# casys-kaist/CoVA

Measured on AMD Instinct MI355X. Metric: compressed-domain frames/sec (BlobNet+bboxcc) at 1080p b=256, higher is better.
Workload: dtype f16

## Files before the change

### cova_amd/csrc/blobnet.h

```cpp
#pragma once
#include <hip/hip_fp16.h>

#include <vector>

#include "internal.h"

constexpr int BN_T = 4;
constexpr int BN_LEVELS = 4;
constexpr int BN_KTAB_STACKS = 256;

struct BnLevelGeom {
    int H, W;
};

struct BnWorkspace {
    bool ready = false;
    __half *act[BN_LEVELS + 1] = {};
    __half *dact[BN_LEVELS] = {};
    __half *pbuf = nullptr;
    size_t pbuf_frames = 0;
    float *part = nullptr;
    int32_t *d_index = nullptr;
    int32_t *h_index = nullptr;
    size_t index_ints = 0;
    hipEvent_t ev_index = nullptr;
    std::vector<int32_t> last_table;
    int last_n_frames = 0;
};

struct covahip_blobnet {
    int H = 0, W = 0, max_batch = 0;
    BnLevelGeom lv[BN_LEVELS + 1];
    int enc_c[BN_LEVELS + 1] = {3, 16, 32, 64, 128};
    int dec_ci[BN_LEVELS] = {128, 128, 64, 32};
    int dec_co[BN_LEVELS] = {64, 32, 16, 16};
    int dec_cy[BN_LEVELS], dec_cx[BN_LEVELS];
    BnWorkspace ws[COVAHIP_MAX_LANES];
    void *d_prepared = nullptr;
    size_t prepared_bytes = 0;
    struct Prepared *prep = nullptr;
    int fuse_tail = 1;
    int fuse_dec = 1;
    int enc1_tile16 = 1;
    int tail_rows = 1;
    int tail_part = 1;
    int fuse_enc23 = 1;
    int enc_rowtiles = 1;
    int64_t macs_per_frame = 0;
};

constexpr int BN_E1_MAXW = 62;
inline bool bn_level1_on_enc1(const covahip_ctx *ctx, const covahip_blobnet *m) {
    return m->enc1_tile16 && m->enc_c[1] == 16 && m->enc_c[2] == 32 && m->lv[1].W <= BN_E1_MAXW && m->lv[1].H >= 2 &&
           !ctx->enc_plan[1].nbands;
}

int blobnet_prepare_mfma(covahip_ctx *ctx, covahip_blobnet *m, const float *h_weights);
void blobnet_release_mfma(covahip_ctx *ctx, covahip_blobnet *m);
struct BnCcTail {
    int area_thresh, max_boxes;
    covahip_box *boxes;
    int32_t *counts;
};
struct BnInput {
    const uint8_t *stack = nullptr;
    const uint8_t *frames = nullptr;
    int n_frames = 0;
    const int32_t *index = nullptr;
    const int32_t *h_index = nullptr;
    bool packed = false;
    bool dry = false;
};
int blobnet_forward_mfma(covahip_ctx *ctx, covahip_blobnet *m, BnWorkspace &ws, const BnInput &in, int batch, float *d_logits,
                         uint8_t *d_mask, const BnCcTail *cc = nullptr, bool *cc_done = nullptr);
```

### cova_amd/csrc/blobnet.hip

```cpp
#include <algorithm>
#include <cstdlib>
#include <cstring>
#include <vector>

#include "blobnet.h"
#include "covahip_dev.h"

namespace {

constexpr uint32_t W_MAGIC = 0x57485643;
constexpr size_t N_PARAMS = 320305;

}

static void free_model(covahip_ctx *ctx, covahip_blobnet *m) {
    if (!m) return;
    blobnet_release_mfma(ctx, m);
    for (BnWorkspace &ws : m->ws) {
        for (int i = 0; i <= BN_LEVELS; i++)
            if (ws.act[i]) hipFree(ws.act[i]);
        for (int j = 0; j < BN_LEVELS; j++)
            if (ws.dact[j]) hipFree(ws.dact[j]);
        if (ws.pbuf) hipFree(ws.pbuf);
        if (ws.part) hipFree(ws.part);
// ... 180 lines not shown
        plan.n_frames = (pass & 2) ? b + BN_T - 1 : 0;
        rc = blobnet_forward_mfma(ctx, m, m->ws[0], plan, b, nullptr, nullptr, nullptr, nullptr);
    }
    return rc;
}

extern "C" {

int covahip_blobnet_load(covahip_ctx *ctx, const void *weights, size_t weights_bytes, int h_mb, int w_mb, int t,
                         int max_batch) {
    if (!ctx || !weights || h_mb <= 0 || w_mb <= 0 || max_batch <= 0) return COVAHIP_ERR_INVALID_ARG;
    if (t != BN_T) return COVAHIP_ERR_UNSUPPORTED;
    if (h_mb < 16 || w_mb < 16 || h_mb > 1024 || w_mb > 1024) return COVAHIP_ERR_UNSUPPORTED;
    if (weights_bytes < 64) return COVAHIP_ERR_BAD_WEIGHTS;
    uint32_t hdr[16];
    std::memcpy(hdr, weights, 64);
    static const uint32_t want[] = {W_MAGIC, 1, 4, 3, 16, 32, 64, 128, 64, 32, 16, 16, (uint32_t)N_PARAMS};
    for (int i = 0; i < 13; i++)
        if (hdr[i] != want[i]) return COVAHIP_ERR_BAD_WEIGHTS;
    if (weights_bytes != 64 + N_PARAMS * sizeof(float)) return COVAHIP_ERR_BAD_WEIGHTS;
    const float *h_w = reinterpret_cast<const float *>(static_cast<const uint8_t *>(weights) + 64);

    COVAHIP_CHECK_HIP(ctx, hipSetDevice(ctx->device));
    covahip_blobnet_destroy(ctx);
    covahip_blobnet *m = new covahip_blobnet();
    int rc = build_model(ctx, m, h_w, h_mb, w_mb, max_batch);
    if (rc == COVAHIP_OK && hipStreamSynchronize(ctx->stream) != hipSuccess) rc = COVAHIP_ERR_HIP;
    if (rc) {
        hipStreamSynchronize(ctx->stream);
        (void)hipGetLastError();
        free_model(ctx, m);
        return rc;
    }
    ctx->blobnet = m;
    return COVAHIP_OK;
}

int covahip_blobnet_macs_per_frame(covahip_ctx *ctx, int64_t *macs) {
    if (!ctx || !macs) return COVAHIP_ERR_INVALID_ARG;
    if (!ctx->blobnet) return COVAHIP_ERR_NOT_LOADED;
    *macs = ctx->blobnet->macs_per_frame;
    return COVAHIP_OK;
}

int covahip_blobnet_set_enc_plan(covahip_ctx *ctx, int level, int nbands, int nbuf) {
    if (!ctx || level < 1 || level > 3 || nbands < 0 || nbands > 64 || (nbands && nbuf != 1 && nbuf != 2)) return COVAHIP_ERR_INVALID_ARG;
    ctx->enc_plan[level].nbands = nbands;
    ctx->enc_plan[level].nbuf = nbands ? nbuf : 0;
    return COVAHIP_OK;
}

int covahip_blobnet_set_impl(covahip_ctx *ctx, int impl) {
    if (!ctx || !ctx->blobnet) return COVAHIP_ERR_NOT_LOADED;
    if (impl != 1 && (impl < 4 || impl > 10)) return COVAHIP_ERR_INVALID_ARG;
    ctx->blobnet->fuse_dec = impl != 4;
    ctx->blobnet->enc1_tile16 = impl != 5;
    ctx->blobnet->enc_rowtiles = impl != 6;
    ctx->blobnet->fuse_enc23 = impl == 7 ? 0 : impl == 8 ? 2 : 1;
    ctx->blobnet->tail_part = impl != 9;
    ctx->blobnet->tail_rows = impl != 10;
    return COVAHIP_OK;
}

static int filter_placed(covahip_ctx *ctx, covahip_blobnet *m, const uint8_t *d_src, int n_frames, const int32_t *stack_index,
                         int batch, int area_thresh, covahip_box *d_boxes, int32_t *d_counts, int max_boxes, float *d_logits,
                         uint8_t *d_mask, bool packed = false) {
    if (!d_mask) {
        CtxLane &l = ctx->lane();
        int rc = covahip_ensure_buffer(ctx, &l.cc_scratch, &l.cc_scratch_bytes, (size_t)batch * m->H * m->W);
        if (rc) return rc;
        d_mask = (uint8_t *)l.cc_scratch;
    }
    BnInput in;
    if (n_frames > 0) {
        int rc = prepare_frames(ctx, m, m->ws[ctx->cur_lane], d_src, n_frames, stack_index, batch, in);
        if (rc) return rc;
        in.packed = packed;
    } else {
        in.stack = d_src;
    }
    return filter_dev(ctx, in, batch, d_logits, d_mask, true, area_thresh, d_boxes, d_counts, max_boxes);
}

static int filter_any(covahip_ctx *ctx, const uint8_t *src, int n_frames, const int32_t *stack_index, int batch,
                      int area_thresh, covahip_box *boxes, int32_t *counts, int max_boxes, float *logits, uint8_t *mask,
                      int mem_kind) {
    if (!ctx || batch < 0 || max_boxes < 0 || n_frames < 0) return COVAHIP_ERR_INVALID_ARG;
    covahip_blobnet *m = ctx->blobnet;
    if (!m) return COVAHIP_ERR_NOT_LOADED;
    if (batch == 0) return COVAHIP_OK;
    if (!src || !counts || (!boxes && max_boxes > 0) || batch > m->max_batch) return COVAHIP_ERR_INVALID_ARG;
    COVAHIP_CHECK_HIP(ctx, hipSetDevice(ctx->device));
    const bool by_frames = n_frames > 0;
    const size_t hw = (size_t)m->H * m->W;
    const size_t in_bytes = by_frames ? (size_t)n_frames * hw * 4 : (size_t)batch * BN_T * hw * 4;
    const size_t mask_bytes = (size_t)batch * hw;
    const size_t logit_bytes = mask_bytes * sizeof(float);
    const size_t box_bytes = (size_t)batch * max_boxes * sizeof(covahip_box);
    const size_t cnt_bytes = (size_t)batch * sizeof(int32_t);
    auto al = [](size_t x) { return (x + 255) & ~(size_t)255; };
    if (mem_kind != COVAHIP_MEM_DEVICE && mem_kind != COVAHIP_MEM_HOST) return COVAHIP_ERR_INVALID_ARG;

    if (mem_kind == COVAHIP_MEM_DEVICE) {
        LaneScope lane(ctx);
        if (!lane.ok()) return COVAHIP_ERR_HIP;
        return filter_placed(ctx, m, src, n_frames, stack_index, batch, area_thresh, boxes, counts, max_boxes, logits, mask);
    }
    if (int rc = covahip_primary_op(ctx)) return rc;
    const uint8_t *d_src = src;
    int rc = covahip_ensure_buffer(ctx, &ctx->stage_in, &ctx->stage_in_bytes, in_bytes);
    if (rc) return rc;
    rc = covahip_ensure_buffer(ctx, &ctx->stage_out, &ctx->stage_out_bytes,
                               al(mask_bytes) + al(logit_bytes) + al(box_bytes) + al(cnt_bytes));
// ... 170 lines not shown
```

### cova_amd/csrc/blobnet_mfma.hip

```cpp
#include <algorithm>
#include <cmath>
#include <cstdlib>
#include <cstring>
#include <mutex>
#include <type_traits>
#include <utility>
#include <vector>

#include "bboxcc_body.h"
#include "bboxcc_wave.h"
#include "blobnet.h"

typedef _Float16 half8 __attribute__((ext_vector_type(8)));
typedef _Float16 half4 __attribute__((ext_vector_type(4)));
typedef float f32x16 __attribute__((ext_vector_type(16)));
typedef float f32x4 __attribute__((ext_vector_type(4)));
typedef _Float16 half2v __attribute__((ext_vector_type(2)));

namespace {

constexpr float BN_EPS = 1e-3f;
constexpr int WG = 256;

struct EncPrep {
// ... 685 lines not shown
        }
        landed();
        PHASE_MARK(6);
#ifdef WGSPAN_ONLY
        ITEM_MARK(3);
        it_n_++;
#endif
    }
#ifdef WGSPAN_ONLY
    if (tid == 0 && blockIdx.x < 1024)
        for (int i = 0; i < 4; i++)
            for (int j = 0; j < 4; j++) g_itemspan[COUT == 32 ? 0 : COUT == 64 ? 1 : 2][blockIdx.x][i][j] = it_t_[i][j];
#endif
#ifdef PHASE_TIMING
#ifndef PHASE_WAVE
#define PHASE_WAVE 0
#endif
    if (tid == 64 * (PHASE_WAVE < 0 ? NWV + PHASE_WAVE : PHASE_WAVE))
        for (int i = 0; i < 9; i++) atomicAdd(&g_phase[i + (PRE ? 0 : COUT == 64 ? 16 : COUT == 128 ? 32 : 48)], ph_[i]);
#endif
    WGSPAN_END(COUT == 32 ? 0 : COUT == 64 ? 1 : 2);
}

constexpr int E2_TSZ = 16384, E3_TSZ = 26112;
constexpr int E1_RS = 2176;
constexpr int E1_TR = 8;
constexpr int E1_TSZ = E1_RS * E1_TR;
constexpr int E1_MAXW = BN_E1_MAXW;
static_assert(8 * 2 * (E1_MAXW + 2) <= 2 * 512 && (E1_MAXW + 2) * 32 + 32 <= E1_RS, "enc1_mfma's staging / row limits");
struct Enc1Args {
    const __half *in;
    __half *out;
    const half8 *wfrag;
    const float *epi;
    int B, H, W, Hp, Wp, Ho, Wo, oy, ox;
    int nbands;
    uint32_t mWp, mRC;
    int scr_off;
    ItemPlan plan;
    const int32_t *pidx;
    __half *skip;
    const float *tm_pre;
    int use_ktab;
    float *part;
    const half8 *wtail;
    uint32_t mXe;
    uint16_t ktab[BN_KTAB_STACKS * BN_T];
};
constexpr int E1_CONST = 2560;
#ifndef E1_ABL
#define E1_ABL 0
#endif
template <bool ALLPOS>
__global__ __launch_bounds__(512, 4) void enc1_mfma(Enc1Args p) {
    constexpr int NWV = 8, WGS = NWV * 64, MG = NWV;
    constexpr int AD = 4;
    extern __shared__ __attribute__((aligned(16))) uint8_t smem[];
    WGSPAN_BEGIN();
    const int tid = threadIdx.x;
    const int wave = __builtin_amdgcn_readfirstlane(tid >> 6);
    for (int i = tid; i < BN_T * E1_TSZ / 16; i += WGS) *reinterpret_cast<uint4 *>(smem + i * 16) = make_uint4(0, 0, 0, 0);
    uint8_t *const cst = smem + p.scr_off + NWV * 1024;
    if (tid < 96) reinterpret_cast<float *>(cst)[tid] = p.epi[tid];
    if (p.part && tid >= 256 && tid < 384) reinterpret_cast<half8 *>(cst + 512)[tid - 256] = p.wtail[tid - 256];
    if (tid >= 128 && tid < 136) {
        const int i = tid & 3;
        const float *tmw = (tid & 4) ? p.tm_pre : p.epi + 96;
        {
            half4 a1, a2;
#pragma unroll
            for (int t = 0; t < BN_T; t++) { a1[t] = (_Float16)tmw[t * BN_T + i]; a2[t] = (_Float16)tmw[16 + t * BN_T + i]; }
            *reinterpret_cast<half4 *>(cst + 384 + (tid & 4) * 16 + i * 16) = a1;
            *reinterpret_cast<half4 *>(cst + 384 + (tid & 4) * 16 + i * 16 + 8) = a2;
        }
    }
    const int RCr = 2 * (p.W + 2);
    const uint32_t plane = (uint32_t)p.H * p.W * 32;
#ifdef PHASE_TIMING
    unsigned long long ph_[9] = {0, 0, 0, 0, 0, 0, 0, 0, 0}, last_ = __builtin_amdgcn_s_memrealtime();
    asm volatile("s_waitcnt lgkmcnt(0)" ::: "memory");
#endif

    ItemIter it;
    for (bool more = it.start(p.plan, p.B, p.nbands); more; more = it.next(p.plan, p.B, p.nbands)) {
        const int b = it.b, band = it.band;
        const int y0 = 2 * ((band * p.Hp) / p.nbands);
        const int rows = 2 * (((band + 1) * p.Hp) / p.nbands) - y0;
        const int n2 = rows + 2;
        auto lane_id = []() -> int {
            uint32_t zero = 0;
            asm volatile("" : "+v"(zero));
            return (int)__builtin_amdgcn_mbcnt_hi(~0u, __builtin_amdgcn_mbcnt_lo(~0u, zero));
        };
        const int ll = lane_id();
        int fidx[BN_T] = {BN_T * b, BN_T * b + 1, BN_T * b + 2, BN_T * b + 3};
        const uint8_t *const fbase = reinterpret_cast<const uint8_t *>(p.in);
        if (p.use_ktab) {
            typedef unsigned u32x2 __attribute__((ext_vector_type(2)));
            typedef const __attribute__((address_space(4))) u32x2 *const_u32x2_ptr;
            const __attribute__((address_space(4))) uint8_t *ka = (const __attribute__((address_space(4))) uint8_t *)__builtin_amdgcn_kernarg_segment_ptr();
            const u32x2 row = *(const_u32x2_ptr)(ka + offsetof(Enc1Args, ktab) + (size_t)b * 8);
            fidx[0] = row[0] & 0xFFFF; fidx[1] = row[0] >> 16; fidx[2] = row[1] & 0xFFFF; fidx[3] = row[1] >> 16;
        } else if (p.pidx) {
            typedef int i32x4 __attribute__((ext_vector_type(4)));
            typedef const __attribute__((address_space(4))) i32x4 *const_i32x4_ptr;
            const i32x4 row = *(const_i32x4_ptr)(uintptr_t)(p.pidx + b * BN_T);
            fidx[0] = row[0]; fidx[1] = row[1]; fidx[2] = row[2]; fidx[3] = row[3];
// ... 185 lines not shown
                __builtin_amdgcn_sched_group_barrier(0x008, 2, 0);
                if (k + AD < 20) __builtin_amdgcn_sched_group_barrier(0x100, 1, 0);
            }
#if E1_ABL == 3
            asm volatile("" :: "v"(tw.x), "v"(e0[0]), "v"(e1[0]), "v"(e0[1]), "v"(e1[1]));
            continue;
#endif
#ifdef PHASE_TIMING
            asm volatile("" : "+v"(pooled[0]), "+v"(pooled[1]));
            PHASE_MARK(6);
#endif
            TmixW tm;
            tm.a1 = __builtin_bit_cast(half4, make_uint2(tw.x, tw.y));
            tm.a2 = __builtin_bit_cast(half4, make_uint2(tw.z, tw.w));
#pragma unroll
            for (int t = 0; t < BN_T; t++) tm.id[t] = (_Float16)(t == (m & 3) ? 1.f : 0.f);
            half4 pb2[2], o2[2];
#pragma unroll
            for (int nt = 0; nt < 2; nt++) pb2[nt] = __builtin_convertvector(pooled[nt], half4);
            tmix4h<2>(tm, pb2, o2);
#pragma unroll
            for (int nt = 0; nt < 2; nt++) {
                _Float16 *sw = reinterpret_cast<_Float16 *>(scr + kg * 256) + nt * 16 + m;
#pragma unroll
                for (int t = 0; t < BN_T; t++) sw[t * 32] = o2[nt][t];
            }
            __builtin_amdgcn_fence(__ATOMIC_RELEASE, "wavefront");
            __builtin_amdgcn_wave_barrier();
            __builtin_amdgcn_fence(__ATOMIC_ACQUIRE, "wavefront");
            const int owin = tile * 4 + kg;
            const uint4 sv = *reinterpret_cast<const uint4 *>(scr + ll * 16);
            if (owin < nwin) {
                const int owy = fdiv(owin, p.mWp), owx = owin - owy * p.Wp;
                const int gy = y0 / 2 + owy + p.oy, gx = owx + p.ox;
                const uint32_t eo = (uint32_t)((gy * p.Wo + gx) * 32 + 8 * (m & 3));
                *reinterpret_cast<uint4 *>(ob + (m >> 2) * tstride + eo) = sv;
                if (ride && m < 4) {
                    float *const pw = reinterpret_cast<float *>(pb4 + (y0 + 2 * owy) * GW + 2 * owx) + m;
                    pw[0] = pride[0]; pw[4] = pride[1]; pw[4 * GW] = pride[2]; pw[4 * GW + 4] = pride[3];
                }
            }
            __builtin_amdgcn_fence(__ATOMIC_RELEASE, "wavefront");
            __builtin_amdgcn_wave_barrier();
            PHASE_MARK(7);
        }
    }
#ifdef PHASE_TIMING
    if (tid == 64 * (PHASE_WAVE < 0 ? NWV + PHASE_WAVE : PHASE_WAVE))
        for (int i = 0; i < 9; i++) atomicAdd(&g_phase[i], ph_[i]);
#endif
    WGSPAN_END(0);
}

constexpr int E23_RP2 = 2048;
constexpr int E23_NSLOT = 6;
constexpr int E23_TSZ2 = E23_NSLOT * E23_RP2;
struct Enc23Args {
    const __half *in;
    __half *mid;
    __half *out;
    const half8 *wf2, *wf3;
    const float *epi2, *epi3;
    int B;
    int H2, W2, Hp2, Wp2;
    int H3, W3, Hp3, Wp3, oy3, ox3;
    int H4, W4, oy4, ox4;
    Swz swz2, swz3;
    int ring_off, xchg_off, scr_off;
};
template <bool AP2, bool AP3>
__global__ __launch_bounds__(512, 2) void enc23_mfma(Enc23Args p) {
    extern __shared__ __attribute__((aligned(256))) uint8_t smem[];
    WGSPAN_BEGIN();
    const int tid = threadIdx.x, lane = tid & 63;
    const int wave = __builtin_amdgcn_readfirstlane(tid >> 6);
    uint8_t *const ring = smem + p.ring_off;
    uint8_t *const xchg = smem + p.xchg_off;
    const int TC3 = p.W3 + 2;
    bool first = true;
    const int tc2 = wave & 1, nt2 = (wave >> 1) & 1, th = wave >> 2;
    const int nt3 = wave & 3, mg3 = wave >> 2;
    for (int b = blockIdx.x; b < p.B; b += gridDim.x) {
        int ll = lane;
        asm volatile("" : "+v"(ll));
        lds_barrier();
        const uint8_t *const src_b = reinterpret_cast<const uint8_t *>(p.in) + (size_t)b * BN_T * p.H2 * p.W2 * 64;
        const int st_t = tid >> 7, st_i = tid & 127, st_c = st_i >> 2, st_x = st_c - 1;
        const bool st_xin = st_x >= 0 && st_x < p.W2;
        uint32_t st_so[2];
#pragma unroll
        for (int k = 0; k < 2; k++)
            st_so[k] = (uint32_t)((min(max(st_x, 0), p.W2 - 1)) * 64 + (((st_i & 3) ^ swz_eval<4>(p.swz2, st_c, k)) << 4));
        const uint8_t *const st_src = src_b + (size_t)st_t * p.H2 * p.W2 * 64;
        uint8_t *const st_dst = ring + st_t * E23_TSZ2 + st_i * 16;
        auto load_rows = [&](int r0, uint4 (&v)[2]) {
#pragma unroll
            for (int k = 0; k < 2; k++) {
                const int rc = min(max(r0 + k, 0), p.H2 - 1);
                v[k] = *reinterpret_cast<const uint4 *>(st_src + (size_t)rc * p.W2 * 64 + st_so[k]);
            }
        };
        auto store_rows = [&](int r0, const uint4 (&v)[2]) {
#pragma unroll
            for (int k = 0; k < 2; k++) {
                const int row = r0 + k;
                const bool in = st_xin && row >= 0 && row < p.H2;
// ... 1286 lines not shown
                else LAUNCH((enc0p_mfma<false, true>), dim3(grid), dim3(WG0), lds, ctx->stream, a);
            } else {
                if (pr->allpos[0]) LAUNCH((enc0p_mfma<true, false>), dim3(grid), dim3(WG0), lds, ctx->stream, a);
                else LAUNCH((enc0p_mfma<false, false>), dim3(grid), dim3(WG0), lds, ctx->stream, a);
            }
        }
        COVAHIP_CHECK_HIP(ctx, hipGetLastError());
    }
    for (int i = 1; i < BN_LEVELS; i++) {
        const int H = m->lv[i].H, W = m->lv[i].W, Hp = H / 2, Wp = W / 2;
        const int cin = m->enc_c[i];
        if (i == 2 && m->fuse_enc23 && m->enc_rowtiles && !ctx->enc_plan[2].nbands && !ctx->enc_plan[3].nbands && cin == 32 &&
            m->enc_c[3] == 64 && m->enc_c[4] == 128) {
            const int H3 = m->lv[3].H, W3 = m->lv[3].W, Hp3 = H3 / 2, Wp3 = W3 / 2;
            const size_t lds = (size_t)BN_T * E3_TSZ + (size_t)BN_T * E23_TSZ2 + 4096;
            const bool pays = 4 * batch >= 3 * num_cu && 20 * Wp >= 17 * 8 * ((Wp + 7) / 8) && 20 * Wp3 >= 17 * 8 * ((Wp3 + 7) / 8);
            if ((pays || m->fuse_enc23 == 2) && (W + 2) * 64 <= E23_RP2 && Wp <= 16 && Hp >= 1 && Hp3 >= 1 && Wp3 >= 1 &&
                (size_t)std::max(2 * Hp3 + 2, H3 + 1) * (W3 + 2) * 128 <= (size_t)E3_TSZ && lds <= 160 * 1024 - 256) {
                Enc23Args a;
                a.in = act[2]; a.mid = act[3]; a.out = act[4];
                a.wf2 = (const half8 *)(prep + pr->enc[2].wfrag); a.wf3 = (const half8 *)(prep + pr->enc[3].wfrag);
                a.epi2 = (const float *)(prep + pr->enc[2].epi); a.epi3 = (const float *)(prep + pr->enc[3].epi);
                a.B = batch;
                a.H2 = H; a.W2 = W; a.Hp2 = Hp; a.Wp2 = Wp;
                a.H3 = H3; a.W3 = W3; a.Hp3 = Hp3; a.Wp3 = Wp3; a.oy3 = H & 1; a.ox3 = W & 1;
                a.H4 = m->lv[4].H; a.W4 = m->lv[4].W; a.oy4 = H3 & 1; a.ox4 = W3 & 1;
                a.swz2 = choose_swz_periodic(32, 30, Wp); a.swz3 = choose_swz_periodic(64, W3, Wp3);
                a.ring_off = BN_T * E3_TSZ; a.xchg_off = a.ring_off + BN_T * E23_TSZ2; a.scr_off = a.ring_off;
                const bool ap2 = pr->allpos[2], ap3 = pr->allpos[3];
                int rc = ap2 ? (ap3 ? set_lds(ctx, enc23_mfma<true, true>, lds) : set_lds(ctx, enc23_mfma<true, false>, lds))
                             : (ap3 ? set_lds(ctx, enc23_mfma<false, true>, lds) : set_lds(ctx, enc23_mfma<false, false>, lds));
                if (rc) return rc;
                const int grid = std::min(batch, num_cu);
                ProfScope ps(ctx, "enc23_mfma");
                if (ap2 && ap3) LAUNCH((enc23_mfma<true, true>), dim3(grid), dim3(512), lds, ctx->stream, a);
                else if (ap2) LAUNCH((enc23_mfma<true, false>), dim3(grid), dim3(512), lds, ctx->stream, a);
                else if (ap3) LAUNCH((enc23_mfma<false, true>), dim3(grid), dim3(512), lds, ctx->stream, a);
                else LAUNCH((enc23_mfma<false, false>), dim3(grid), dim3(512), lds, ctx->stream, a);
                COVAHIP_CHECK_HIP(ctx, hipGetLastError());
                break;
            }
        }
        if (i == 1 && bn_level1_on_enc1(ctx, m)) {
            const long long slots = 2LL * num_cu;
            long long best = -1;
            int nbands = 0;
            for (int nb = 1; nb <= Hp; nb++) {
                const int rb = (Hp + nb - 1) / nb;
                if (2 * rb + 2 > E1_TR) continue;
                const long long rounds = ((long long)batch * nb + slots - 1) / slots;
                const long long cost = rounds * (rb + 1);
                if (best < 0 || cost < best) { best = cost; nbands = nb; }
            }
            if (nbands) {
                Enc1Args a;
                a.in = ws.pbuf; a.out = act[2];
                a.wfrag = (const half8 *)(prep + pr->enc1w); a.epi = (const float *)(prep + pr->enc[1].epi);
                a.B = batch; a.H = H; a.W = W; a.Hp = Hp; a.Wp = Wp; a.Ho = m->lv[2].H; a.Wo = m->lv[2].W;
                a.oy = H & 1; a.ox = W & 1; a.nbands = nbands;
                a.mWp = magic(Wp); a.mRC = magic(2 * (W + 2));
                a.scr_off = BN_T * E1_TSZ;
                const int grid = std::min(batch * nbands, 2 * num_cu);
                a.plan = make_plan(grid, num_cu, 2, batch, nbands, Hp);
                a.pidx = d_index; a.skip = act[1]; a.tm_pre = (const float *)(prep + pr->enc[0].epi) + 48;
                part_written = m->tail_part && ws.part && m->dec_ci[3] == 32 && m->dec_co[3] == 16 && m->enc_c[1] == 16;
                a.part = part_written ? ws.part : nullptr;
                a.wtail = (const half8 *)(prep + pr->tail_w);
                a.mXe = magic(2 * Wp);
                a.use_ktab = 0;
                if (by_frames && inp.h_index && batch <= BN_KTAB_STACKS) {
                    a.use_ktab = 1;
                    for (int k = 0; k < batch * BN_T; k++) a.ktab[k] = (uint16_t)inp.h_index[k];
                } else if (by_frames && !d_index && !dry) {
                    return COVAHIP_ERR_INVALID_ARG;
                }
                const size_t lds = (size_t)BN_T * E1_TSZ + 8 * 1024 + E1_CONST;
                int rc = pr->allpos[1] ? set_lds(ctx, enc1_mfma<true>, lds) : set_lds(ctx, enc1_mfma<false>, lds);
                if (rc) return rc;
                ProfScope ps(ctx, "enc1_mfma");
                if (pr->allpos[1]) LAUNCH(enc1_mfma<true>, dim3(grid), dim3(512), lds, ctx->stream, a);
                else LAUNCH(enc1_mfma<false>, dim3(grid), dim3(512), lds, ctx->stream, a);
                COVAHIP_CHECK_HIP(ctx, hipGetLastError());
                continue;
            }
        }
        const size_t px_bytes = (size_t)cin * 2;
        const int TC = W + 2;
        static const int enc_waves[BN_LEVELS] = {0, 8, 4, 8};
        int waves = enc_waves[i], nbuf = 1, wgs_per_cu = (i == BN_LEVELS - 1) ? 1 : 2;
        int nbands = 0, RB = 0;
        size_t scr_bytes = (size_t)waves * 2048;
        if (ctx->enc_plan[i].nbands) {
            nbands = std::min(ctx->enc_plan[i].nbands, Hp);
            nbuf = ctx->enc_plan[i].nbuf;
            RB = 2 * ((Hp + nbands - 1) / nbands);
            const size_t need = (size_t)nbuf * BN_T * (RB + 2) * TC * px_bytes + scr_bytes;
            if (need > 160 * 1024 - 256) return COVAHIP_ERR_UNSUPPORTED;
            wgs_per_cu = (i == BN_LEVELS - 1) ? 1 : (int)std::min<size_t>(2, (160 * 1024 - 256) / need);
        } else {
            const size_t lds_cap = (wgs_per_cu == 1 ? 150 * 1024 : 80 * 1024) - scr_bytes;
            const long long slots = (long long)wgs_per_cu * num_cu;
            long long best = -1;
            for (int nb = 1; nb <= Hp; nb++) {
                const int rb = (Hp + nb - 1) / nb;
                if ((size_t)BN_T * (2 * rb + 2) * TC * px_bytes > lds_cap) continue;
                const long long rounds = ((long long)batch * nb + slots - 1) / slots;
                const long long cost = rounds * (rb + 1);
                if (best < 0 || cost < best) { best = cost; nbands = nb; RB = 2 * rb; }
            }
            if (!nbands) return COVAHIP_ERR_UNSUPPORTED;
        }
        const int fix_tsz = i == 2 ? E2_TSZ : i == 3 ? E3_TSZ : 0;
        bool rowtiles = false;
        if (fix_tsz && m->enc_rowtiles && !ctx->enc_plan[i].nbands && cin == (i == 2 ? 32 : 64) && m->enc_c[i + 1] == 2 * cin &&
            (size_t)(RB + 2) * TC * px_bytes <= (size_t)fix_tsz) {
            long long t_rows = (long long)Hp * ((Wp + 7) / 8), t_gen = 0;
            for (int k = 0; k < nbands; k++) t_gen += ((((k + 1) * Hp) / nbands - (k * Hp) / nbands) * Wp + 7) / 8;
            rowtiles = t_rows <= t_gen;
        }
        const size_t tile_bytes = rowtiles ? (size_t)BN_T * fix_tsz : (((size_t)BN_T * (RB + 2) * TC * px_bytes) + 15) & ~(size_t)15;
        const size_t lds = nbuf * tile_bytes + scr_bytes;
        if (lds > 160 * 1024 - 256) return COVAHIP_ERR_UNSUPPORTED;
        const int items = batch * nbands;
        const int grid = std::min(items, wgs_per_cu * num_cu);
        EncArgs a;
        a.in = i == 1 ? ws.pbuf : act[i]; a.out = act[i + 1];
        a.wfrag = (const half8 *)(prep + pr->enc[i].wfrag); a.epi = (const float *)(prep + pr->enc[i].epi);
        a.B = batch; a.H = H; a.W = W; a.Hp = Hp; a.Wp = Wp; a.Ho = m->lv[i + 1].H; a.Wo = m->lv[i + 1].W;
        a.oy = H & 1; a.ox = W & 1; a.To = (i == BN_LEVELS - 1) ? 1 : BN_T;
        a.RB = RB; a.nbands = nbands; a.TR = RB + 2; a.TC = TC;
        a.mWp = magic(Wp); a.mNb = magic(nbands); a.mRC = magic(TC * (cin / 8)); a.zero = prep + pr->zero;
        a.nbuf = nbuf; a.buf_stride = (int)tile_bytes; a.scr_off = (int)(nbuf * tile_bytes);
        a.plan = make_plan(grid, num_cu, wgs_per_cu, batch, nbands, Hp);
        a.swz = rowtiles ? choose_swz_periodic(cin, W, Wp) : choose_swz(true, cin, W, Wp, RB / 2);
// ... 224 lines not shown
```

### cova_amd/elements.py

```python
from __future__ import annotations

import ctypes as C

import numpy as np

from . import _lib as L
from . import weights as W

FLOW_OK = "ok"
FLOW_DROPPED = "dropped"


def _ptr(a: np.ndarray) -> int:
    return a.ctypes.data


class Context:

    def __init__(self, device_id: int = 0):
        self._lib = L.lib()
        h = C.c_void_p()
        L.check(self._lib.covahip_ctx_create(device_id, C.byref(h)), "covahip_ctx_create")
        self.handle = h
        self.device_id = device_id
# ... 71 lines not shown

    def __init__(self, timestep: int = 1, gamma: int = 1):
        self.timestep = timestep
        self.gamma = gamma
        self._h = None
        self._lib = L.lib()

    def transform_caps(self, width: int, height: int):
        ow, oh = C.c_int(), C.c_int()
        self._lib.covahip_stack_out_dims(width, height, self.timestep, C.byref(ow), C.byref(oh))
        return ow.value, oh.value

    def set_caps(self, width: int, height: int):
        ow, oh = self.transform_caps(width, height)
        out_size = ow * oh * 4
        self.size_per_buf = out_size // self.timestep
        self.out_size = out_size
        self.stop()
        h = C.c_void_p()
        L.check(self._lib.covahip_stack_new(self.size_per_buf, self.timestep, self.gamma, C.byref(h)), "stack_new")
        self._h = h
        return ow, oh

    def transform(self, inbuf: bytes | np.ndarray):
        a = np.frombuffer(inbuf, dtype=np.uint8) if not isinstance(inbuf, np.ndarray) else inbuf.reshape(-1)
        a = np.ascontiguousarray(a, dtype=np.uint8)
        out = np.empty(self.out_size, dtype=np.uint8)
        em = C.c_int()
        L.check(self._lib.covahip_stack_push(self._h, _ptr(a), a.size, _ptr(out), out.size, C.byref(em)), "stack_push")
        return (FLOW_OK, out) if em.value else (FLOW_DROPPED, None)

    def stop(self):
        if self._h:
            self._lib.covahip_stack_free(self._h)
            self._h = None

    __del__ = stop


class BlobNetInfer:

    def __init__(self, ctx: Context, weights_flat: np.ndarray, h_mb: int, w_mb: int, max_batch: int,
                 timestep: int = 4):
        self.ctx, self.h, self.w, self.t, self.max_batch = ctx, h_mb, w_mb, timestep, max_batch
        self._lib = L.lib()
        blob = W.to_bytes(weights_flat)
        L.check(self._lib.covahip_blobnet_load(ctx.handle, blob, len(blob), h_mb, w_mb, timestep, max_batch),
                "covahip_blobnet_load", ctx.handle)

    def set_enc_plan(self, level: int, nbands: int, nbuf: int = 1):
        L.check(self._lib.covahip_blobnet_set_enc_plan(self.ctx.handle, level, nbands, nbuf), "covahip_blobnet_set_enc_plan")

    def set_impl(self, impl: str):
        L.check(self._lib.covahip_blobnet_set_impl(self.ctx.handle, {"mfma": 1, "dec_separate": 4, "enc1_legacy": 5, "enc_general_tiles": 6, "enc23_separate": 7, "enc23_force": 8, "tail_skip_tensor": 9, "tail_band_tiles": 10}[impl]), "set_impl")

    def read_buffer(self, which: int, index: int = 0) -> np.ndarray:
        p, n, dims = C.c_void_p(), C.c_size_t(), (C.c_int32 * 5)()
        L.check(self._lib.covahip_dev_blobnet_buffer(self.ctx.handle, which, index, C.byref(p), C.byref(n), dims),
                "covahip_dev_blobnet_buffer", self.ctx.handle)
        out = np.empty(tuple(d for d in dims if d), dtype=np.float32 if which == 3 else np.float16)
        assert p.value and out.nbytes == n.value, (which, index, n.value, tuple(dims))
        self.ctx.d2h(out, p.value)
        return out

    @property
    def macs_per_frame(self) -> int:
        v = C.c_int64()
        L.check(self._lib.covahip_blobnet_macs_per_frame(self.ctx.handle, C.byref(v)), "macs_per_frame")
        return v.value

    def infer(self, stack: np.ndarray, want_logits: bool = True):
        stack = np.ascontiguousarray(stack, dtype=np.uint8)
        b = stack.shape[0]
        assert stack.shape == (b, self.t * self.h, self.w, 4), stack.shape
        logits = np.empty((b, self.h, self.w), dtype=np.float32) if want_logits else None
        mask = np.empty((b, self.h, self.w), dtype=np.uint8)
        L.check(self._lib.covahip_blobnet_forward(self.ctx.handle, _ptr(stack), b, _ptr(logits) if want_logits else None,
                                                  _ptr(mask), L.MEM_HOST), "covahip_blobnet_forward", self.ctx.handle)
        return logits, mask

    def infer_device(self, d_stack: int, batch: int, d_logits: int | None, d_mask: int | None):
        L.check(self._lib.covahip_blobnet_forward(self.ctx.handle, d_stack, batch, d_logits, d_mask, L.MEM_DEVICE),
                "covahip_blobnet_forward", self.ctx.handle)

    def filter(self, stack: np.ndarray, cc_threshold: int, max_boxes: int = 256, want_mask: bool = False):
        stack = np.ascontiguousarray(stack, dtype=np.uint8)
        b = stack.shape[0]
        boxes = np.zeros((b, max_boxes), dtype=L.BOX_DTYPE)
        counts = np.zeros(b, dtype=np.int32)
        mask = np.empty((b, self.h, self.w), dtype=np.uint8) if want_mask else None
        L.check(self._lib.covahip_filter_forward(self.ctx.handle, _ptr(stack), b, cc_threshold, _ptr(boxes), _ptr(counts),
                                                 max_boxes, None, _ptr(mask) if want_mask else None, L.MEM_HOST),
                "covahip_filter_forward", self.ctx.handle)
        return boxes, counts, mask

    def filter_frames(self, frames: np.ndarray, stack_index: np.ndarray | None, cc_threshold: int, max_boxes: int = 256,
                      want_mask: bool = False, want_logits: bool = False):
        frames = np.ascontiguousarray(frames, dtype=np.uint8)
        f = frames.shape[0]
        assert frames.shape == (f, self.h, self.w, 4), frames.shape
        idx = None if stack_index is None else np.ascontiguousarray(stack_index, dtype=np.int32).reshape(-1, 4)
        b = f - 3 if idx is None else idx.shape[0]
        boxes = np.zeros((b, max_boxes), dtype=L.BOX_DTYPE)
        counts = np.zeros(b, dtype=np.int32)
        mask = np.empty((b, self.h, self.w), dtype=np.uint8) if want_mask else None
        logits = np.empty((b, self.h, self.w), dtype=np.float32) if want_logits else None
        L.check(self._lib.covahip_filter_forward_frames(self.ctx.handle, _ptr(frames), f, None if idx is None else _ptr(idx), b,
# ... 430 lines not shown
```

Measured before the change: 2.394 million.

## Add warp-specialized ring-buffer enc1 kernel with persistent per-stack pipelining

Adds a new enc1 path using 1024-thread workgroups split into compute waves and staging waves. The staging waves prefetch and temporal-mix input rows into a 10-row LDS ring while the compute waves run the MFMA conv+pool on earlier rows. Workgroups are persistent over stacks (grid = min(batch, CUs)), and the next stack's first rows are prefetched at the end of each one. The path is on by default when batch is large relative to CU count. This is meant to hide global-load latency and remove the band-split halo overhead, at the cost of a more complex kernel, heavier LDS and register use, and lower occupancy.

```diff
diff --git a/cova_amd/csrc/blobnet.h b/cova_amd/csrc/blobnet.h
--- a/cova_amd/csrc/blobnet.h
+++ b/cova_amd/csrc/blobnet.h
@@ -43,6 +43,7 @@
     int fuse_dec = 1;
     int enc1_tile16 = 1;
     int tail_rows = 1;
+    int enc1_ring = 1;
     int tail_part = 1;
     int fuse_enc23 = 1;
     int enc_rowtiles = 1;
diff --git a/cova_amd/csrc/blobnet.hip b/cova_amd/csrc/blobnet.hip
--- a/cova_amd/csrc/blobnet.hip
+++ b/cova_amd/csrc/blobnet.hip
@@ -256,13 +256,14 @@
 
 int covahip_blobnet_set_impl(covahip_ctx *ctx, int impl) {
     if (!ctx || !ctx->blobnet) return COVAHIP_ERR_NOT_LOADED;
-    if (impl != 1 && (impl < 4 || impl > 10)) return COVAHIP_ERR_INVALID_ARG;
+    if (impl != 1 && (impl < 4 || impl > 12)) return COVAHIP_ERR_INVALID_ARG;
     ctx->blobnet->fuse_dec = impl != 4;
     ctx->blobnet->enc1_tile16 = impl != 5;
     ctx->blobnet->enc_rowtiles = impl != 6;
     ctx->blobnet->fuse_enc23 = impl == 7 ? 0 : impl == 8 ? 2 : 1;
     ctx->blobnet->tail_part = impl != 9;
     ctx->blobnet->tail_rows = impl != 10;
+    ctx->blobnet->enc1_ring = impl == 11 ? 0 : impl == 12 ? 2 : 1;
     return COVAHIP_OK;
 }
 
diff --git a/cova_amd/csrc/blobnet_mfma.hip b/cova_amd/csrc/blobnet_mfma.hip
--- a/cova_amd/csrc/blobnet_mfma.hip
+++ b/cova_amd/csrc/blobnet_mfma.hip
@@ -761,7 +761,7 @@
 #define E1_ABL 0
 #endif
 template <bool ALLPOS>
-__global__ __launch_bounds__(512, 4) void enc1_mfma(Enc1Args p) {
+__device__ __forceinline__ void enc1_bands(const Enc1Args &p) {
     constexpr int NWV = 8, WGS = NWV * 64, MG = NWV;
     constexpr int AD = 4;
     extern __shared__ __attribute__((aligned(16))) uint8_t smem[];
@@ -1053,6 +1053,342 @@
     WGSPAN_END(0);
 }
 
+constexpr int E1R_ROWS = 10;
+constexpr int E1R_TSZ = E1_RS * E1R_ROWS;
+constexpr int E1R_NWV = 16, E1R_NTW = 8;
+constexpr int E1R_AD = 4;
+constexpr int E1R_MLPN = 2;
+constexpr int E1R_NPC = (4 * 2 * (E1_MAXW + 2) + (E1R_NWV - E1R_NTW) * 64 - 1) / ((E1R_NWV - E1R_NTW) * 64);
+static_assert(6 * 2 * (E1_MAXW + 2) <= E1R_NWV * 64, "enc1_ring: one staged piece per lane (a stack's first six rows)");
+static_assert(3 * E1R_TSZ + 64 < 65536, "enc1_ring: fragment offsets fit a ds_read's immediate");
+struct E1Piece {
+    half8 v[BN_T];
+    int dst;
+    uint32_t eoff;
+    bool inb, have;
+};
+__device__ __forceinline__ void e1_frames(const Enc1Args &p, int b, int (&fidx)[BN_T]) {
+    fidx[0] = BN_T * b; fidx[1] = BN_T * b + 1; fidx[2] = BN_T * b + 2; fidx[3] = BN_T * b + 3;
+    if (p.use_ktab) {
+        typedef unsigned u32x2 __attribute__((ext_vector_type(2)));
+        typedef const __attribute__((address_space(4))) u32x2 *const_u32x2_ptr;
+        const __attribute__((address_space(4))) uint8_t *ka = (const __attribute__((address_space(4))) uint8_t *)__builtin_amdgcn_kernarg_segment_ptr();
+        const u32x2 row = *(const_u32x2_ptr)(ka + offsetof(Enc1Args, ktab) + (size_t)b * 8);
+        fidx[0] = row[0] & 0xFFFF; fidx[1] = row[0] >> 16; fidx[2] = row[1] & 0xFFFF; fidx[3] = row[1] >> 16;
+    } else if (p.pidx) {
+        typedef int i32x4 __attribute__((ext_vector_type(4)));
+        typedef const __attribute__((address_space(4))) i32x4 *const_i32x4_ptr;
+        const i32x4 row = *(const_i32x4_ptr)(uintptr_t)(p.pidx + b * BN_T);
+        fidx[0] = row[0]; fidx[1] = row[1]; fidx[2] = row[2]; fidx[3] = row[3];
+    }
+}
+__device__ __forceinline__ void e1r_issue(const Enc1Args &p, const int (&fidx)[BN_T], int i, int R0, int nr, E1Piece &q) {
+    const int RCr = 2 * (p.W + 2), nreal = nr * RCr;
+    const uint32_t plane = (uint32_t)p.H * p.W * 32;
+    const int ic = min(i, nreal - 1);
+    const int r = fdiv(ic, p.mRC), within = ic - r * RCr;
+    const int c = within >> 1, hf = within & 1;
+    const int y = R0 + r - 1, x = c - 1;
+    int slot = R0 % E1R_ROWS + r;
+    slot -= slot >= E1R_ROWS ? E1R_ROWS : 0;
+    q.inb = y >= 0 && y < p.H && x >= 0 && x < p.W;
+    q.dst = slot * E1_RS + c * 32 + hf * 16;
+    q.eoff = (uint32_t)((min(max(y, 0), p.H - 1) * p.W + min(max(x, 0), p.W - 1)) * 32 + hf * 16);
+    q.have = i < nreal;
+    const uint8_t *const fbase = reinterpret_cast<const uint8_t *>(p.in);
+#pragma unroll
+    for (int t = 0; t < BN_T; t++) {
+        const uint64_t fo = (uint64_t)(uint32_t)fidx[t] * plane;
+        const uint32_t lo = __builtin_amdgcn_readfirstlane((uint32_t)fo), hi = __builtin_amdgcn_readfirstlane((uint32_t)(fo >> 32));
+        q.v[t] = *reinterpret_cast<const half8 *>(fbase + (((uint64_t)hi << 32) | lo) + q.eoff);
+    }
+}
+__device__ __forceinline__ void e1r_land(const Enc1Args &p, uint8_t *smem, const uint8_t *cst, int ll, int b, E1Piece &q) {
+    if (!q.inb) {
+#pragma unroll
+        for (int t = 0; t < BN_T; t++)
+#pragma unroll
+            for (int j = 0; j < 8; j++) q.v[t][j] = (_Float16)0;
+    }
+    TmixW tmp;
+    {
+        const uint4 w = *reinterpret_cast<const uint4 *>(cst + 448 + (ll & 3) * 16);
+        tmp.a1 = __builtin_bit_cast(half4, make_uint2(w.x, w.y));
+        tmp.a2 = __builtin_bit_cast(half4, make_uint2(w.z, w.w));
+#pragma unroll
+        for (int t = 0; t < BN_T; t++) tmp.id[t] = (_Float16)(t == (ll & 3) ? 1.f : 0.f);
+    }
+    half8 o[BN_T];
+#pragma unroll
+    for (int j0 = 0; j0 < 8; j0 += E1R_MLPN) {
+        half4 pb[E1R_MLPN];
+        f32x4 rr[E1R_MLPN];
+#pragma unroll
+        for (int j = 0; j < E1R_MLPN; j++) pb[j] = half4{q.v[0][j0 + j], q.v[1][j0 + j], q.v[2][j0 + j], q.v[3][j0 + j]};
+        tmix4f<E1R_MLPN>(tmp, pb, rr);
+#pragma unroll
+        for (int j = 0; j < E1R_MLPN; j++)
+#pragma unroll
+            for (int t = 0; t < BN_T; t++) o[t][j0 + j] = (_Float16)rr[j][t];
+    }
+    if (q.have) {
+#pragma unroll
+        for (int t = 0; t < BN_T; t++) *reinterpret_cast<half8 *>(smem + t * E1R_TSZ + q.dst) = o[t];
+    }
+    if (q.have && q.inb && !p.part)
+        *reinterpret_cast<half8 *>(reinterpret_cast<uint8_t *>(p.skip) + (size_t)b * BN_T * p.H * p.W * 32 + q.eoff) = o[0];
+}
+template <bool ALLPOS>
+__device__ __forceinline__ void enc1_ring(const Enc1Args &p) {
+    constexpr int NWV = E1R_NWV, NTW = E1R_NTW, NSW = NWV - NTW, NPC = E1R_NPC;
+    constexpr int AD = E1R_AD;
+    extern __shared__ __attribute__((aligned(16))) uint8_t smem[];
+    WGSPAN_BEGIN();
+    const int tid = threadIdx.x;
+    const int wave = __builtin_amdgcn_readfirstlane(tid >> 6);
+    const int ll = [] {
+        uint32_t zero = 0;
+        asm volatile("" : "+v"(zero));
+        return (int)__builtin_amdgcn_mbcnt_hi(~0u, __builtin_amdgcn_mbcnt_lo(~0u, zero));
+    }();
+    const int m = ll & 15, kg = ll >> 4;
+    const int nsteps = (p.Hp + 1) / 2;
+    uint8_t *const cst = smem + p.scr_off + NWV * 1024;
+    const bool ride = p.part != nullptr;
+    const int GW = p.W + 1;
+
+    int b = blockIdx.x;
+    {
+        int fidx[BN_T];
+        E1Piece q;
+        e1_frames(p, b, fidx);
+        e1r_issue(p, fidx, tid, 0, 6, q);
+        for (int i = tid; i < BN_T * E1R_TSZ / 16; i += NWV * 64) *reinterpret_cast<uint4 *>(smem + i * 16) = make_uint4(0, 0, 0, 0);
+        if (tid < 96) reinterpret_cast<float *>(cst)[tid] = p.epi[tid];
+        if (p.part && tid >= 256 && tid < 384) reinterpret_cast<half8 *>(cst + 512)[tid - 256] = p.wtail[tid - 256];
+        if (tid >= 128 && tid < 136) {
+            const int i = tid & 3;
+            const float *tmw = (tid & 4) ? p.tm_pre : p.epi + 96;
+            half4 a1, a2;
+#pragma unroll
+            for (int t = 0; t < BN_T; t++) { a1[t] = (_Float16)tmw[t * BN_T + i]; a2[t] = (_Float16)tmw[16 + t * BN_T + i]; }
+            *reinterpret_cast<half4 *>(cst + 384 + (tid & 4) * 16 + i * 16) = a1;
+            *reinterpret_cast<half4 *>(cst + 384 + (tid & 4) * 16 + i * 16 + 8) = a2;
+        }
+        lds_barrier();
+        e1r_land(p, smem, cst, ll, b, q);
+    }
+    auto restart = [&](int bn) {
+        lds_barrier();
+        int fidx[BN_T];
+        E1Piece q;
+        e1_frames(p, bn, fidx);
+        e1r_issue(p, fidx, tid, 0, 6, q);
+        e1r_land(p, smem, cst, ll, bn, q);
+    };
+
+    if (wave < NTW) {
+        uint8_t *const scr = smem + p.scr_off + wave * 1024;
+        const uint32_t tstride = (uint32_t)(p.Ho * p.Wo * 32);
+        half8 bf[2][5];
+        {
+            const half8 *wp = p.wfrag + ll;
+            asm volatile("" : "+v"(wp));
+#pragma unroll
+            for (int nt = 0; nt < 2; nt++)
+#pragma unroll
+                for (int s = 0; s < 5; s++) bf[nt][s] = wp[(nt * 5 + s) * 64];
+        }
+        lds_barrier();
+        for (;;) {
+            const int bn = b + (int)gridDim.x;
+            f32x4 *const pb4 = reinterpret_cast<f32x4 *>(p.part) + (size_t)b * (p.H + 1) * GW;
+            __half *const ob = p.out + (size_t)b * BN_T * tstride;
+            int R0m = 0;
+            for (int s = 0; s < nsteps; s++) {
+                const int nwin = min(2, p.Hp - 2 * s) * p.Wp;
+                const int ntiles = (nwin + 3) / 4;
+                for (int tile = wave; tile < ntiles; tile += NTW) {
+                    const int win = min(tile * 4 + (m >> 2), nwin - 1);
+                    const int wy = fdiv(win, p.mWp), wx = win - wy * p.Wp;
+                    const int yy0 = 2 * wy + ((m >> 1) & 1), xx0 = 2 * wx + (m & 1);
+                    auto rowoff = [&](int d) {
+                        int q = R0m + yy0 + d;
+                        q -= q >= E1R_ROWS ? E1R_ROWS : 0;
+                        return q * E1_RS;
+                    };
+                    const int cb = xx0 * 32 + (kg & 1) * 16;
+                    const int r0 = rowoff(0), r1 = rowoff(1), r2 = rowoff(2);
+                    const uint8_t *const aH0 = smem + r0 + cb + (kg >> 1) * 32, *const aH1 = smem + r1 + cb + (kg >> 1) * 32,
+                                         *const aH2 = smem + r2 + cb + (kg >> 1) * 32, *const aV = smem + ((kg >> 1) ? r1 : r0) + cb + 64;
+                    auto frag = [&](int idx) -> half8 {
+                        const int s = (idx % 10) >> 1, t = 2 * (idx / 10) + (idx & 1);
+                        const uint8_t *a = s == 3 ? aV : s == 4 ? aH2 + 64 : s == 0 ? aH0 : s == 1 ? aH1 : aH2;
+                        return *reinterpret_cast<const half8 *>(__builtin_assume_aligned(a + t * E1R_TSZ, 16));
+                    };
+                    half8 ab[AD];
+#pragma unroll
+                    for (int k = 0; k < AD; k++) ab[k] = frag(k);
+                    const float *cf = reinterpret_cast<const float *>(cst);
+                    float e0[2], e1[2], e2[2];
+#pragma unroll
+                    for (int nt = 0; nt < 2; nt++) {
+                        e0[nt] = cf[nt * 16 + m]; e1[nt] = cf[32 + nt * 16 + m];
+                        e2[nt] = ALLPOS ? 0.f : cf[64 + nt * 16 + m];
+                    }
+                    f32x4 acc[2][2];
+                    f32x4 pooled[2];
+                    const f32x4 z4 = {0.f, 0.f, 0.f, 0.f};
+                    f32x4 pride = z4;
+#pragma unroll
+                    for (int k = 0; k < 20; k++) {
+                        const int s = (k % 10) >> 1, tp = k & 1;
+#pragma unroll
+                        for (int nt = 0; nt < 2; nt++)
+                            acc[nt][tp] = __builtin_amdgcn_mfma_f32_16x16x32_f16(ab[k % AD], bf[nt][s], s == 0 ? z4 : acc[nt][tp], 0, 0, 0);
+                        if ((k == 0 || k == 2) && ride)
+                            pride = __builtin_amdgcn_mfma_f32_16x16x32_f16(ab[k % AD], *reinterpret_cast<const half8 *>(cst + 512 + (k >> 1) * 1024 + ll * 16),
+                                                                           pride, 0, 0, 0);
+                        if (k + AD < 20) ab[k % AD] = frag(k + AD);
+                        if (s == 4) {
+#pragma unroll
+                            for (int nt = 0; nt < 2; nt++) {
+                                float pv = pool4<ALLPOS>(acc[nt][tp][0], acc[nt][tp][1], acc[nt][tp][2], acc[nt][tp][3], e0[nt], e1[nt], e2[nt]);
+                                asm volatile("" : "+v"(pv));
+                                pooled[nt][2 * (k / 10) + tp] = pv;
+                            }
+                        }
+                    }
+                    __builtin_amdgcn_sched_group_barrier(0x100, AD, 0);
+#pragma unroll
+                    for (int k = 0; k < 20; k++) {
+                        __builtin_amdgcn_sched_group_barrier(0x008, 2, 0);
+                        if (k + AD < 20) __builtin_amdgcn_sched_group_barrier(0x100, 1, 0);
+                    }
+                    const uint4 tw = *reinterpret_cast<const uint4 *>(cst + 384 + (m & 3) * 16);
+                    TmixW tm;
+                    tm.a1 = __builtin_bit_cast(half4, make_uint2(tw.x, tw.y));
+                    tm.a2 = __builtin_bit_cast(half4, make_uint2(tw.z, tw.w));
+#pragma unroll
+                    for (int t = 0; t < BN_T; t++) tm.id[t] = (_Float16)(t == (m & 3) ? 1.f : 0.f);
+                    half4 pb2[2], o2[2];
+#pragma unroll
+                    for (int nt = 0; nt < 2; nt++) pb2[nt] = __builtin_convertvector(pooled[nt], half4);
+                    tmix4h<2>(tm, pb2, o2);
+#pragma unroll
+                    for (int nt = 0; nt < 2; nt++) {
+                        _Float16 *sw = reinterpret_cast<_Float16 *>(scr + kg * 256) + nt * 16 + m;
+#pragma unroll
+                        for (int t = 0; t < BN_T; t++) sw[t * 32] = o2[nt][t];
+                    }
+                    __builtin_amdgcn_fence(__ATOMIC_RELEASE, "wavefront");
+                    __builtin_amdgcn_wave_barrier();
+                    __builtin_amdgcn_fence(__ATOMIC_ACQUIRE, "wavefront");
+                    const int owin = tile * 4 + kg;
+                    const uint4 sv = *reinterpret_cast<const uint4 *>(scr + ll * 16);
+                    if (owin < nwin) {
+                        const int owy = fdiv(owin, p.mWp), owx = owin - owy * p.Wp;
+                        const int gy = 2 * s + owy + p.oy, gx = owx + p.ox;
+                        const uint32_t eo = (uint32_t)((gy * p.Wo + gx) * 32 + 8 * (m & 3));
+                        *reinterpret_cast<uint4 *>(ob + (m >> 2) * tstride + eo) = sv;
+                        if (ride && m < 4) {
+                            float *const pw = reinterpret_cast<float *>(pb4 + (4 * s + 2 * owy) * GW + 2 * owx) + m;
+                            pw[0] = pride[0]; pw[4] = pride[1]; pw[4 * GW] = pride[2]; pw[4 * GW + 4] = pride[3];
+                        }
+                    }
+                    __builtin_amdgcn_fence(__ATOMIC_RELEASE, "wavefront");
+                    __builtin_amdgcn_wave_barrier();
+                }
+                if (s == nsteps - 1 && bn < p.B) restart(bn);
+                lds_barrier();
+                R0m += 4;
+                R0m -= R0m >= E1R_ROWS ? E1R_ROWS : 0;
+            }
+            if (bn >= p.B) break;
+            b = bn;
+        }
+    } else {
+        const int j = (wave - NTW) * 64 + ll;
+        int fidx[BN_T];
+        E1Piece qa[NPC];
+        e1_frames(p, b, fidx);
+        if (nsteps > 1)
+#pragma unroll
+            for (int k = 0; k < NPC; k++) e1r_issue(p, fidx, j + k * NSW * 64, 6, 4, qa[k]);
+        lds_barrier();
+        for (;;) {
+            const int bn = b + (int)gridDim.x;
+            f32x4 *const pb4 = reinterpret_cast<f32x4 *>(p.part) + (size_t)b * (p.H + 1) * GW;
+            int R0m = 0;
+            for (int s = 0; s < nsteps; s++) {
+                const bool last = s == nsteps - 1;
+                if (!last) {
+#pragma unroll
+                    for (int k = 0; k < NPC; k++) e1r_land(p, smem, cst, ll, b, qa[k]);
+                    if (s + 2 < nsteps)
+#pragma unroll
+                        for (int k = 0; k < NPC; k++) e1r_issue(p, fidx, j + k * NSW * 64, 4 * s + 10, 4, qa[k]);
+                }
+                if (ride) {
+                    const int y0 = 4 * s, rows = 2 * min(2, p.Hp - 2 * s);
+                    const int ub = last ? p.H + 1 : y0 + rows;
+                    const int xe = 2 * p.Wp, ce = GW - xe;
+                    const int ne1 = (ub - y0) * ce;
+                    const int ne2 = max(0, ub - (y0 + rows)) * xe;
+                    const int npos = ne1 + ne2;
+                    const int nptiles = (npos + 15) / 16;
+                    if (wave - NTW < nptiles) {
+                        const half8 w0 = *reinterpret_cast<const half8 *>(cst + 512 + ll * 16), w1 = *reinterpret_cast<const half8 *>(cst + 1536 + ll * 16);
+                        for (int pt = wave - NTW; pt < nptiles; pt += NSW) {
+                            const int q = pt * 16 + m;
+                            const int qc = min(q, npos - 1);
+                            int u, vv;
+                            if (qc < ne1) {
+                                const int ul = ce == 1 ? qc : qc >> 1;
+                                u = y0 + ul; vv = xe + (qc - ul * ce);
+                            } else {
+                                const int q2 = qc - ne1, ul = fdiv(q2, p.mXe);
+                                u = y0 + rows + ul; vv = q2 - ul * xe;
+                            }
+                            int s1 = R0m + (u - y0);
+                            s1 -= s1 >= E1R_ROWS ? E1R_ROWS : 0;
+                            const int s0 = s1 + 1 == E1R_ROWS ? 0 : s1 + 1;
+                            const int col = (vv + (kg >> 1)) * 32 + (kg & 1) * 16;
+                            const int o1 = s1 * E1_RS + col;
+                            const int o0 = u >= p.H ? 0 : s0 * E1_RS + col;
+                            const half8 b1 = *reinterpret_cast<const half8 *>(__builtin_assume_aligned(smem + o1, 16));
+                            const half8 b0 = *reinterpret_cast<const half8 *>(__builtin_assume_aligned(smem + o0, 16));
+                            const f32x4 z4 = {0.f, 0.f, 0.f, 0.f};
+                            f32x4 pe = __builtin_amdgcn_mfma_f32_16x16x32_f16(w0, b1, z4, 0, 0, 0);
+                            pe = __builtin_amdgcn_mfma_f32_16x16x32_f16(w1, b0, pe, 0, 0, 0);
+                            if (kg == 0 && q < npos) pb4[u * GW + vv] = pe;
+                        }
+                    }
+                }
+                if (last && bn < p.B) {
+                    restart(bn);
+                    e1_frames(p, bn, fidx);
+                    if (nsteps > 1)
+#pragma unroll
+                        for (int k = 0; k < NPC; k++) e1r_issue(p, fidx, j + k * NSW * 64, 6, 4, qa[k]);
+                }
+                lds_barrier();
+                R0m += 4;
+                R0m -= R0m >= E1R_ROWS ? E1R_ROWS : 0;
+            }
+            if (bn >= p.B) break;
+            b = bn;
+        }
+    }
+    WGSPAN_END(0);
+}
+
+template <bool ALLPOS, bool RING>
+__global__ __launch_bounds__(RING ? 1024 : 512, 4) void enc1_mfma(Enc1Args p) {
+    if constexpr (RING) enc1_ring<ALLPOS>(p);
+    else enc1_bands<ALLPOS>(p);
+}
+
 constexpr int E23_RP2 = 2048;
 constexpr int E23_NSLOT = 6;
 constexpr int E23_TSZ2 = E23_NSLOT * E23_RP2;
@@ -2445,16 +2781,17 @@
                 const long long cost = rounds * (rb + 1);
                 if (best < 0 || cost < best) { best = cost; nbands = nb; }
             }
-            if (nbands) {
+            const bool ring = m->enc1_ring == 2 || (m->enc1_ring == 1 && 4 * batch >= 3 * num_cu);
+            if (ring || nbands) {
                 Enc1Args a;
                 a.in = ws.pbuf; a.out = act[2];
                 a.wfrag = (const half8 *)(prep + pr->enc1w); a.epi = (const float *)(prep + pr->enc[1].epi);
                 a.B = batch; a.H = H; a.W = W; a.Hp = Hp; a.Wp = Wp; a.Ho = m->lv[2].H; a.Wo = m->lv[2].W;
                 a.oy = H & 1; a.ox = W & 1; a.nbands = nbands;
                 a.mWp = magic(Wp); a.mRC = magic(2 * (W + 2));
-                a.scr_off = BN_T * E1_TSZ;
-                const int grid = std::min(batch * nbands, 2 * num_cu);
-                a.plan = make_plan(grid, num_cu, 2, batch, nbands, Hp);
+                a.scr_off = ring ? BN_T * E1R_TSZ : BN_T * E1_TSZ;
+                const int grid = ring ? std::min(batch, num_cu) : std::min(batch * nbands, 2 * num_cu);
+                if (!ring) a.plan = make_plan(grid, num_cu, 2, batch, nbands, Hp);
                 a.pidx = d_index; a.skip = act[1]; a.tm_pre = (const float *)(prep + pr->enc[0].epi) + 48;
                 part_written = m->tail_part && ws.part && m->dec_ci[3] == 32 && m->dec_co[3] == 16 && m->enc_c[1] == 16;
                 a.part = part_written ? ws.part : nullptr;
@@ -2467,12 +2804,21 @@
                 } else if (by_frames && !d_index && !dry) {
                     return COVAHIP_ERR_INVALID_ARG;
                 }
-                const size_t lds = (size_t)BN_T * E1_TSZ + 8 * 1024 + E1_CONST;
-                int rc = pr->allpos[1] ? set_lds(ctx, enc1_mfma<true>, lds) : set_lds(ctx, enc1_mfma<false>, lds);
-                if (rc) return rc;
-                ProfScope ps(ctx, "enc1_mfma");
-                if (pr->allpos[1]) LAUNCH(enc1_mfma<true>, dim3(grid), dim3(512), lds, ctx->stream, a);
-                else LAUNCH(enc1_mfma<false>, dim3(grid), dim3(512), lds, ctx->stream, a);
+                if (ring) {
+                    const size_t lds = (size_t)BN_T * E1R_TSZ + E1R_NWV * 1024 + E1_CONST;
+                    int rc = pr->allpos[1] ? set_lds(ctx, enc1_mfma<true, true>, lds) : set_lds(ctx, enc1_mfma<false, true>, lds);
+                    if (rc) return rc;
+                    ProfScope ps(ctx, "enc1_mfma");
+                    if (pr->allpos[1]) LAUNCH((enc1_mfma<true, true>), dim3(grid), dim3(E1R_NWV * 64), lds, ctx->stream, a);
+                    else LAUNCH((enc1_mfma<false, true>), dim3(grid), dim3(E1R_NWV * 64), lds, ctx->stream, a);
+                } else {
+                    const size_t lds = (size_t)BN_T * E1_TSZ + 8 * 1024 + E1_CONST;
+                    int rc = pr->allpos[1] ? set_lds(ctx, enc1_mfma<true, false>, lds) : set_lds(ctx, enc1_mfma<false, false>, lds);
+                    if (rc) return rc;
+                    ProfScope ps(ctx, "enc1_mfma");
+                    if (pr->allpos[1]) LAUNCH((enc1_mfma<true, false>), dim3(grid), dim3(512), lds, ctx->stream, a);
+                    else LAUNCH((enc1_mfma<false, false>), dim3(grid), dim3(512), lds, ctx->stream, a);
+                }
                 COVAHIP_CHECK_HIP(ctx, hipGetLastError());
                 continue;
             }
diff --git a/cova_amd/elements.py b/cova_amd/elements.py
--- a/cova_amd/elements.py
+++ b/cova_amd/elements.py
@@ -147,7 +147,7 @@
         L.check(self._lib.covahip_blobnet_set_enc_plan(self.ctx.handle, level, nbands, nbuf), "covahip_blobnet_set_enc_plan")
 
     def set_impl(self, impl: str):
-        L.check(self._lib.covahip_blobnet_set_impl(self.ctx.handle, {"mfma": 1, "dec_separate": 4, "enc1_legacy": 5, "enc_general_tiles": 6, "enc23_separate": 7, "enc23_force": 8, "tail_skip_tensor": 9, "tail_band_tiles": 10}[impl]), "set_impl")
+        L.check(self._lib.covahip_blobnet_set_impl(self.ctx.handle, {"mfma": 1, "dec_separate": 4, "enc1_legacy": 5, "enc_general_tiles": 6, "enc23_separate": 7, "enc23_force": 8, "tail_skip_tensor": 9, "tail_band_tiles": 10, "enc1_bands": 11, "enc1_ring_force": 12}[impl]), "set_impl")
 
     def read_buffer(self, which: int, index: int = 0) -> np.ndarray:
         p, n, dims = C.c_void_p(), C.c_size_t(), (C.c_int32 * 5)()
```

After: 2.373 million (median of 6 runs). No clear change (-0.9%).
